# Aakash1312/Fluid-Simulation

Measured on AMD Instinct MI355X. Metric: simulated substeps/sec, higher is better.
Workload: dtype f64

## Files before the change

### fluid-simulation_amd/csrc/common.h

```cpp
#pragma once
#include <hip/hip_runtime.h>
#include <stdint.h>

namespace fl {

constexpr uint8_t F_SOLID = 1;
constexpr uint8_t F_FLUID = 2;
constexpr int F_CNT_SHIFT = 2;

struct Grid {
    int N;
    int lo;
    int hi;
    int nx, ny, nz;
    int ox, oy, oz;
    __host__ __device__ inline size_t idx(int ix, int iy, int iz) const
    {
        return ((size_t)ix * ny + (size_t)iy) * nz + (size_t)iz;
    }
    __host__ __device__ inline size_t cells() const { return (size_t)nx * ny * nz; }
    __host__ __device__ inline long sx() const { return (long)ny * nz; }
    __host__ __device__ inline int cx0() const { return lo + ox; }
    __host__ __device__ inline int cy0() const { return lo + oy; }
    __host__ __device__ inline int cz0() const { return lo + oz; }
// ... 167 lines not shown
    __host__ __device__ inline Particles shifted(long o) const
    {
        Particles q = *this;
        q.px += o; q.py += o; q.pz += o; q.vx += o; q.vy += o; q.vz += o; q.pid += o;
        return q;
    }
};
constexpr uint32_t PID_DEAD = 0xFFFFFFFFu;

void launch_bin_count(hipStream_t st, Grid g, long n, Particles p, int* key, int* slot, int* cell_count, int* part, StepState* ss);
void launch_bin_scatter(hipStream_t st, long n, const int* key, const int* slot, const int* cell_start, const uint32_t* pid, int* order,
                         uint32_t* spid);
void launch_bin_rank(hipStream_t st, long n_pos, long pos0, const int* key, const int* cell_start, const int* order, const uint32_t* spid,
                     int* order2);
void launch_reorder(hipStream_t st, long n, const int* order, Particles src, Particles dst, double* w = nullptr, long wstride = 0);
void launch_weights(hipStream_t st, long n, Particles p, double* w, long stride);
void launch_axpby_box(hipStream_t st, Grid g, Box box, double a, const double* x, double b, const double* y, double* out, const PcgState* gate = nullptr);
long p2g_max_items(Box box);
size_t p2g_part_doubles(Box box);
constexpr int P2G_PILED = 256;
void launch_p2g(hipStream_t st, Grid g, Box box, Particles p, const double* pw, long wstride, const int* cell_start, const uint8_t* flags,
                double* part, int* items, float* container, double* u, double* v, double* w, double* ub, double* vb, double* wb, int2* crowd_list = nullptr,
                Particles park = Particles{});
void launch_p2g_tiles(hipStream_t st, Grid g, Box box, Particles p, const double* pw, long wstride, const int* cell_start, const uint8_t* flags,
                      float* container, double* u, double* v, double* w, double* ub, double* vb, double* wb);
void launch_g2p_tiled(hipStream_t st, Grid g, Box pb, Particles p, const int* cell_start, const double* dcx, const double* dcy, const double* dcz,
                      const double* pcx, const double* pcy, const double* pcz, double blend, StepState* ss);
void launch_g2p(hipStream_t st, Grid g, long n, Particles p, const double* dcx, const double* dcy, const double* dcz, const double* pcx,
                const double* pcy, const double* pcz, double blend, StepState* ss);
void launch_advect(hipStream_t st, Grid g, long n, Particles p, const uint8_t* flags, double max_dt, double dx, StepState* ss);
void launch_advect_bin(hipStream_t st, Grid g, long n, Particles p, const uint8_t* flags, double max_dt, double dx, StepState* ss, int* key,
                       int* slot, int* cell_count, int* part);
void launch_pack_particles(hipStream_t st, long n, Particles p, double* pos_aos, double* vel_aos);
void launch_unpack_records(hipStream_t st, long n, const double* rec, Particles p, long off);
void launch_pack_records(hipStream_t st, long n, Particles p, long off, double* rec);
void launch_unpack_ids(hipStream_t st, long n, const double* pos, const double* vel, const uint32_t* ids, Particles p);
void launch_pack_ids(hipStream_t st, long n, Particles p, long off, double* pos, double* vel, uint32_t* ids);
void launch_unpack_particles(hipStream_t st, long n, const double* pos_aos, const double* vel_aos, Particles p);

void launch_out_mark(hipStream_t st, const float* f, int N, int off, int nl, int* flags);
void launch_out_pack(hipStream_t st, const float* f, int N, int lo, int off, int nl, const int* flags, const int* slot, float* values,
                     int* origin);
struct OutWin {
    int ny, nz;
    int ox, oy, oz;
    int olo[3], ohi[3];
    int lo, off;
    int l0[3], nl[3];
    __host__ __device__ inline long leaves() const { return (long)nl[0] * nl[1] * nl[2]; }
};
void launch_out_mark_win(hipStream_t st, const float* f, const OutWin& w, int* flags);
void launch_out_pack_win(hipStream_t st, const float* f, const OutWin& w, const int* flags, const int* slot, float* values, int* origin);
void launch_exclusive_scan(hipStream_t st, const int* in, int* out, long n, int* block_sums, int* total);
void launch_sort_tail(hipStream_t st, const int* cell_count, int* cell_start, long c1, long ncell);
void launch_index_scan(hipStream_t st, Grid g, const uint8_t* flags, int* indices, int* block_sums, int* total);
void launch_index_scan_flat(hipStream_t st, const uint8_t* flags, int* indices, long n, int* block_sums, int* total);
void launch_flags(hipStream_t st, Grid g, const uint8_t* solid, const float* container, uint8_t* flags, int x0, int x1);
void launch_index_scan_range(hipStream_t st, Grid g, const uint8_t* flags, int* indices, int* block_sums, int* total, int x0, int x1);
void launch_rhs_div(hipStream_t st, Grid g, Box box, const uint8_t* flags, const double* u, const double* v, const double* w,
                    float* rhs, float* diver, double dx, double gdt0, double gdt1, double gdt2, bool rows = false, const PcgState* gate = nullptr);
void launch_vel_update(hipStream_t st, Grid g, Box box, const uint8_t* flags, const double* p, double* u, double* v, double* w,
                       double k, double g0, double g1, double g2, bool rows = false, const PcgState* gate = nullptr);
void launch_flip_delta(hipStream_t st, Grid g, Box box, const double* u, const double* v, const double* w,
                       const double* ub, const double* vb, const double* wb, double* dcx, double* dcy, double* dcz, double* pcx, double* pcy, double* pcz);
void launch_err_norm(hipStream_t st, Grid g, Box box, const uint8_t* flags, const float* b, const float* b2, double* part, StepState* ss,
                     const PcgState* gate = nullptr);
void launch_zero_step_state(hipStream_t st, StepState* ss, int N);
struct ZeroList { float* f4[4]; double* f8[7]; };
void launch_zero_fields(hipStream_t st, const ZeroList& z, Grid g, Box box, bool rows = false);
// ... 128 lines not shown
```

### fluid-simulation_amd/csrc/fluid_api.hip

```cpp
#include "sim.h"
#include <algorithm>

using namespace fl;

static thread_local std::string g_err;
int fluid_fail(int code, const std::string& msg)
{
    g_err = msg;
    return code;
}
#define fail fluid_fail

Box fl::clip_dilate(const Box& b, int d, const Grid& g)
{
    Box r;
    r.x0 = b.x0 - d < 0 ? 0 : b.x0 - d;
    r.y0 = b.y0 - d < 0 ? 0 : b.y0 - d;
    r.z0 = b.z0 - d < 0 ? 0 : b.z0 - d;
    r.x1 = b.x1 + d > g.nx - 1 ? g.nx - 1 : b.x1 + d;
    r.y1 = b.y1 + d > g.ny - 1 ? g.ny - 1 : b.y1 + d;
    r.z1 = b.z1 + d > g.nz - 1 ? g.nz - 1 : b.z1 + d;
    return r;
}

// ... 189 lines not shown
    s->prm = *p;
    s->g = g;
    s->ncell = g.cells();
    s->dt = p->max_dt;
    s->mg_fp32 = p->mg_precision == FLUID_MG_FP32;
    s->warm = p->solve_start == FLUID_START_WARM;
    if (const char* e = getenv("FLUID_MG_CSWEEPS")) s->mg_csweeps = atoi(e);
    if (const char* e = getenv("FLUID_TILE_LISTS")) s->lists_force = atoi(e) != 0;
    if (const char* e = getenv("FLUID_P2G_FORM")) s->p2g_force = !strcmp(e, "rows") ? 1 : (!strcmp(e, "tiles") ? 2 : (!strcmp(e, "crowd") ? 3 : 0));
    if (const char* e = getenv("FLUID_MG_GALERKIN")) s->gal_mode = atoi(e);
    if (const char* e = getenv("FLUID_DROPLETS")) s->drops_on = atoi(e) != 0;
    if (const char* e = getenv("FLUID_ROW_SWEEPS")) s->row_sweeps = atoi(e) != 0;
    if (const char* e = getenv("FLUID_DROPLETS_MIN")) s->drop_min = atoi(e);
    if (const char* e = getenv("FLUID_ADVECT_BIN")) s->advect_bin = atoi(e) != 0;
    if (const char* e = getenv("FLUID_SOLVE_TAIL")) s->solve_tail = atoi(e) != 0;
    *out = nullptr;
    auto bail = [&](int rc) { fluid_destroy(s); return rc; };
#define A(expr) do { hipError_t e_ = (expr); if (e_ != hipSuccess) return bail(fail(FLUID_ERR_HIP, std::string(#expr) + ": " + hipGetErrorString(e_))); } while (0)
    A(hipStreamCreateWithFlags(&s->st, hipStreamNonBlocking));
    const size_t n = s->ncell;
    A(dalloc(&s->solid, n)); A(dalloc(&s->flags, n));
    A(dalloc(&s->container, n)); A(dalloc(&s->rhs, n)); A(dalloc(&s->diver, n)); A(dalloc(&s->diver2, n));
    A(dalloc(&s->u, n)); A(dalloc(&s->v, n)); A(dalloc(&s->w, n));
    A(dalloc(&s->ub, n)); A(dalloc(&s->vb, n)); A(dalloc(&s->wb, n));
    A(dalloc(&s->dcx, n)); A(dalloc(&s->dcy, n)); A(dalloc(&s->dcz, n));
    A(dalloc(&s->pressure, n));
    if (s->warm) {
        A(dalloc(&s->p_guess, n)); A(dalloc(&s->p_guess2, n));
        if (hipMemset(s->p_guess, 0, n * sizeof(double)) != hipSuccess || hipMemset(s->p_guess2, 0, n * sizeof(double)) != hipSuccess) return bail(FLUID_ERR_HIP);
        if (const char* e = getenv("FLUID_EXTRAPOLATE")) s->extrapolate = atoi(e) != 0;
        if (s->extrapolate) { A(dalloc(&s->p_q, n)); if (hipMemset(s->p_q, 0, n * sizeof(double)) != hipSuccess) return bail(FLUID_ERR_HIP); }
    }
    A(dalloc(&s->indices, n));
    A(dalloc(&s->scan_sums, (n + 2) / 2048 + 16));
// ... 155 lines not shown
    HIPCHK(hipMemcpyAsync(s->h_ss, s->ss, sizeof(StepState), hipMemcpyDeviceToHost, s->st));
    HIPCHK(hipStreamSynchronize(s->st));
    return FLUID_OK;
}

int fl::clear_dirty(fluid_sim* s)
{
    if (box_empty(s->dirty)) return FLUID_OK;
    const ZeroList z = {{s->container, s->rhs, s->diver, s->diver2}, {s->u, s->v, s->w, s->ub, s->vb, s->wb, s->pressure}};
    launch_zero_fields(s->st, z, s->g, s->dirty, !s->dist && s->row_sweeps);
    HIPCHK(hipGetLastError());
    s->dirty = Box{0, 0, 0, -1, -1, -1};
    return FLUID_OK;
}

int fl::sort_pass(fluid_sim* s, int ax0, int ax1, int* h_tail)
{
    const Grid g = s->g;
    const long ncell = (long)s->ncell, n2 = g.sx();
    const long c0 = (long)ax0 * n2, c1 = (long)(ax1 + 1) * n2;
    launch_zero_step_state(s->st, s->ss, g.N);
    HIPCHK(hipMemsetAsync(s->cell_count + c0, 0, (c1 - c0) * sizeof(int), s->st));
    HIPCHK(hipMemsetAsync(s->cell_count + ncell, 0, 4 * sizeof(int), s->st));
    launch_bin_count(s->st, g, s->np, s->pa.shifted(s->p_off), s->key, s->slot, s->cell_count, s->ipart, s->ss);
    launch_exclusive_scan(s->st, s->cell_count + c0, s->cell_start + c0, c1 - c0, s->scan_sums, s->cell_start + c1);
    launch_sort_tail(s->st, s->cell_count, s->cell_start, c1, ncell);
    launch_bin_scatter(s->st, s->np, s->key, s->slot, s->cell_start, s->pa.shifted(s->p_off).pid, s->order, s->spid);
    launch_bin_rank(s->st, s->np, 0, s->key, s->cell_start, s->order, s->spid, s->order2);
    HIPCHK(hipGetLastError());
    if (h_tail) HIPCHK(hipMemcpyAsync(h_tail, s->cell_start + ncell, 3 * sizeof(int), hipMemcpyDeviceToHost, s->st));
    return read_ss(s);
}

static int sort_binned(fluid_sim* s)
{
    const Grid g = s->g;
    const long ncell = (long)s->ncell, n2 = g.sx();
    const long c0 = (long)s->bin_x0 * n2, c1 = (long)(s->bin_x1 + 1) * n2;
    launch_zero_step_state(s->st, s->ss, g.N);
    launch_exclusive_scan(s->st, s->cell_count + c0, s->cell_start + c0, c1 - c0, s->scan_sums, s->cell_start + c1);
    launch_sort_tail(s->st, s->cell_count, s->cell_start, c1, ncell);
    launch_bin_scatter(s->st, s->np, s->key, s->slot, s->cell_start, s->pa.shifted(s->p_off).pid, s->order, s->spid);
    launch_bin_rank(s->st, s->np, 0, s->key, s->cell_start, s->order, s->spid, s->order2);
    HIPCHK(hipGetLastError());
    StepState& h = *s->h_ss;
    for (int a = 0; a < 3; ++a) h.bbox_min[a] = s->bin_min[a], h.bbox_max[a] = s->bin_max[a];
    h.n_out = s->bin_n_out;
    h.max_cell = s->bin_max_cell;
    return FLUID_OK;
}

static int phase_sort(fluid_sim* s)
{
    const Grid g = s->g;
    int tok = prof_begin(s, FLUID_PROF_SORT, (double)s->np);
    int ax0 = 0, ax1 = g.nx - 1;
    const bool guess = s->sort_hint && !box_empty(s->Pb);
    if (guess) {
// ... 18 lines not shown
    s->sort_hint = true;
    s->n_out = s->h_ss->n_out;
    s->max_cell = s->h_ss->max_cell;
    const StepState& h = *s->h_ss;
    if (h.bbox_max[0] < 0) {
        s->Pb = Box{0, 0, 0, -1, -1, -1};
    } else {
        s->Pb = Box{h.bbox_min[0], h.bbox_min[1], h.bbox_min[2], h.bbox_max[0], h.bbox_max[1], h.bbox_max[2]};
    }
    if (!box_empty(s->Pb)) {
        s->Rb = clip_dilate(s->Pb, 1, g);
        s->Sb = clip_dilate(s->Pb, 2, g);
    } else {
        s->Rb = s->Sb = s->Pb;
    }
    launch_reorder(s->st, s->np, s->order2, s->pa.shifted(s->p_off), s->pb, s->pw, s->cap);
    HIPCHK(hipGetLastError());
    std::swap(s->pa, s->pb);
    s->p_off = 0;
    prof_end(s, FLUID_PROF_SORT, tok);
    s->sorted = true;
    return FLUID_OK;
}

int fl::run_p2g(fluid_sim* s, const Box& box)
{
    const long ref_cells = s->p2g_ref_cells > 0 ? s->p2g_ref_cells : s->Rb.cells();
    const bool airy = s->last_num_active > 0 && (double)s->last_num_active < 0.3 * (double)ref_cells;
    const bool huge = (size_t)12 * sizeof(double) * (size_t)box.cells() > ((size_t)16 << 30);
    const bool piled = s->max_cell > P2G_PILED || airy;
    if (s->p2g_force ? s->p2g_force == 2 : huge) {
// ... 642 lines not shown
        HIPCHK(hipMalloc((void**)q, s->ncell * sizeof(double)));
        HIPCHK(hipMemsetAsync(*q, 0, s->ncell * sizeof(double), s->st));
    }
    return FLUID_OK;
}

static int phase_flip_advect(fluid_sim* s)
{
    if (!s->have_p2g) return fail(FLUID_ERR_STATE, "flip_advect before p2g");
    HIPCHK(hipSetDevice(s->prm.device));
    int rcp = pic_fields(s);
    if (rcp) return rcp;
    if (!box_empty(s->Rb)) launch_flip_delta(s->st, s->g, s->Rb, s->u, s->v, s->w, s->ub, s->vb, s->wb, s->dcx, s->dcy, s->dcz, s->pcx, s->pcy, s->pcz);
    int tok = prof_begin(s, FLUID_PROF_G2P, (double)s->np);
    if (s->sorted && s->p_off == 0 && (double)s->np >= 4.0 * (double)s->Pb.cells()) {
        launch_g2p_tiled(s->st, s->g, s->Pb, s->pa, s->cell_start, s->dcx, s->dcy, s->dcz, s->pcx, s->pcy, s->pcz, s->prm.flip_blend, s->ss);
        if (!box_empty(s->Pb)) s->stats.paths |= FLUID_PATH_G2P_TILES;
        if (s->n_out > 0)
            launch_g2p(s->st, s->g, s->n_out, s->pa.shifted(s->np - s->n_out), s->dcx, s->dcy, s->dcz, s->pcx, s->pcy, s->pcz, s->prm.flip_blend, s->ss);
    } else {
        launch_g2p(s->st, s->g, s->np, s->pa.shifted(s->p_off), s->dcx, s->dcy, s->dcz, s->pcx, s->pcy, s->pcz, s->prm.flip_blend, s->ss);
    }
    prof_end(s, FLUID_PROF_G2P, tok);
    const bool bin = s->advect_bin && !s->dist && s->np > 0 && s->sorted && s->sort_hint && !box_empty(s->Pb);
    s->binned = false;
    if (bin) {
        const Grid g = s->g;
        s->bin_x0 = std::max(0, s->Pb.x0 - 3);
        s->bin_x1 = std::min(g.nx - 1, s->Pb.x1 + 3);
        const long n2 = g.sx(), c0 = (long)s->bin_x0 * n2, c1 = (long)(s->bin_x1 + 1) * n2;
        HIPCHK(hipMemsetAsync(s->cell_count + c0, 0, (c1 - c0) * sizeof(int), s->st));
        HIPCHK(hipMemsetAsync(s->cell_count + s->ncell, 0, 4 * sizeof(int), s->st));
        launch_advect_bin(s->st, g, s->np, s->pa.shifted(s->p_off), s->flags, s->prm.max_dt, s->prm.dx, s->ss, s->key, s->slot, s->cell_count, s->ipart);
    } else {
        launch_advect(s->st, s->g, s->np, s->pa.shifted(s->p_off), s->flags, s->prm.max_dt, s->prm.dx, s->ss);
    }
    HIPCHK(hipGetLastError());
    int rc = read_ss(s);
    if (rc) return rc;
    if (bin) {
        const StepState& h = *s->h_ss;
        for (int a = 0; a < 3; ++a) s->bin_min[a] = h.bbox_min[a], s->bin_max[a] = h.bbox_max[a];
        s->bin_n_out = h.n_out;
        s->bin_max_cell = h.max_cell;
        s->binned = true;
    }
    s->dt = s->h_ss->dt;
// ... 373 lines not shown
```

### fluid-simulation_amd/csrc/fluid_dist.hip

```cpp
#include "sim.h"
#include "dist_kernels.h"

using namespace fl;
#define fail fluid_fail
int cuts_from_hist(int n, const int64_t* hist, int P, int32_t* cuts);

#define COMMCHK(expr)                                                                              \
    do {                                                                                           \
        if ((expr) != 0) return fail(FLUID_ERR_HIP, std::string("comm callback failed: ") + #expr); \
    } while (0)

namespace {

constexpr int HALO_W = 4;

struct IBox {
    int lo[3], hi[3];
};
inline bool ib_empty(const IBox& b) { return b.hi[0] <= b.lo[0] || b.hi[1] <= b.lo[1] || b.hi[2] <= b.lo[2]; }
inline IBox ib_isect(const IBox& a, const IBox& b)
{
    IBox r;
    for (int k = 0; k < 3; ++k) { r.lo[k] = std::max(a.lo[k], b.lo[k]); r.hi[k] = std::min(a.hi[k], b.hi[k]); }
    if (ib_empty(r)) for (int k = 0; k < 3; ++k) { r.lo[k] = a.lo[k]; r.hi[k] = a.lo[k]; }
// ... 398 lines not shown
        s->stats.box_hi[a] = d->Rg.hi[a] - 1;
    }
}

int dist_g2p_advect(fluid_sim* s, fluid_step_stats_t* stats)
{
    DistState* d = s->ds;
    const Grid g = s->g;
    int rc;
    launch_kill_ghosts(s->st, g, d->ob, s->np, s->pa.shifted(s->p_off));
    int tok = prof_begin(s, FLUID_PROF_G2P, (double)s->np);
    const IBox ownb{{d->ob.lo[0], d->ob.lo[1], d->ob.lo[2]}, {d->ob.hi[0], d->ob.hi[1], d->ob.hi[2]}};
    const int org[3] = {g.ox, g.oy, g.oz};
    const Box ownPb = to_box(ib_isect(d->Pg, ownb), org);
    if (s->p_off == 0 && !box_empty(ownPb) && (double)s->np >= 4.0 * (double)ownPb.cells()) {
        launch_g2p_tiled(s->st, g, ownPb, s->pa, s->cell_start, s->dcx, s->dcy, s->dcz, s->pcx, s->pcy, s->pcz, s->prm.flip_blend, s->ss);
        if (s->n_out > 0)
            launch_g2p(s->st, g, s->n_out, s->pa.shifted(s->np - s->n_out), s->dcx, s->dcy, s->dcz, s->pcx, s->pcy, s->pcz, s->prm.flip_blend, s->ss);
    } else {
        launch_g2p(s->st, g, s->np, s->pa.shifted(s->p_off), s->dcx, s->dcy, s->dcz, s->pcx, s->pcy, s->pcz, s->prm.flip_blend, s->ss);
    }
    prof_end(s, FLUID_PROF_G2P, tok);
    HIPCHK(hipGetLastError());
    if ((rc = comm_allreduce(s, &s->ss->max_speed_bits, 1, FLUID_DT_I64, FLUID_OP_MAX))) return rc;
    launch_advect(s->st, g, s->np, s->pa.shifted(s->p_off), s->flags, s->prm.max_dt, s->prm.dx, s->ss);
    HIPCHK(hipGetLastError());
    if ((rc = read_ss(s))) return rc;
    s->dt = s->h_ss->dt;
    double ms;
    memcpy(&ms, &s->h_ss->max_speed_bits, sizeof(double));
    s->stats.max_speed = ms;
// ... 1561 lines not shown
```

### fluid-simulation_amd/csrc/kernels_grid.hip

```cpp
#include "common.h"

namespace fl {

constexpr int SCAN_T = 256;
constexpr int SCAN_E = 8;
constexpr int SCAN_CHUNK = SCAN_T * SCAN_E;

template <int MODE>
__device__ __forceinline__ int scan_load(const void* in, long i)
{
    if (MODE == 0) return ((const int*)in)[i];
    return (((const uint8_t*)in)[i] & F_FLUID) ? 1 : 0;
}

template <int MODE, bool VEC>
__device__ __forceinline__ void scan_load8(const void* in, long base, long n, int v[SCAN_E])
{
    if (VEC && base >= 0 && base + SCAN_E <= n) {
        if (MODE == 0) {
            const int4 a = *(const int4*)((const int*)in + base), b = *(const int4*)((const int*)in + base + 4);
            v[0] = a.x; v[1] = a.y; v[2] = a.z; v[3] = a.w;
            v[4] = b.x; v[5] = b.y; v[6] = b.z; v[7] = b.w;
        } else {
            const uint2 w = *(const uint2*)((const uint8_t*)in + base);
// ... 492 lines not shown
{
    ss->bbox_min[0] = ss->bbox_min[1] = ss->bbox_min[2] = N;
    ss->bbox_max[0] = ss->bbox_max[1] = ss->bbox_max[2] = -1;
    ss->num_active = 0;
    ss->n_out = 0;
    ss->n_drop_fail = 0;
    ss->max_speed_bits = 0ull;
    ss->err_num = 0;
    ss->err_den = 0;
}
void launch_zero_step_state(hipStream_t st, StepState* ss, int N)
{
    hipLaunchKernelGGL(k_zero_step_state, dim3(1), dim3(1), 0, st, ss, N);
}

__global__ void k_sort_tail(const int* __restrict__ cell_count, int* __restrict__ cell_start, long c1, long ncell)
{
    const int t = cell_start[c1];
    cell_start[ncell] = t;
    cell_start[ncell + 1] = t + cell_count[ncell];
    cell_start[ncell + 2] = t + cell_count[ncell] + cell_count[ncell + 1];
}
void launch_sort_tail(hipStream_t st, const int* cell_count, int* cell_start, long c1, long ncell)
{
    hipLaunchKernelGGL(k_sort_tail, dim3(1), dim3(1), 0, st, cell_count, cell_start, c1, ncell);
}

__global__ __launch_bounds__(256) void k_zero_fields(ZeroList z, Grid g, Box box)
{
    const int a = blockIdx.y;
    float* pf = z.f4[0];
#pragma unroll
    for (int q = 1; q < 4; ++q) pf = (a == q) ? z.f4[q] : pf;
    double* pd = z.f8[0];
#pragma unroll
    for (int q = 1; q < 7; ++q) pd = (a - 4 == q) ? z.f8[q] : pd;
    CellIt it = box_cell(g, box);
    if (!it.ok) return;
// ... 170 lines not shown
```

### fluid-simulation_amd/csrc/kernels_particles.hip

```cpp
#include "common.h"

namespace fl {

struct BinAcc {
    int mn[3] = {0x7fffffff, 0x7fffffff, 0x7fffffff}, mx[3] = {-1, -1, -1};
    int nout = 0, cmax = 0;
};
__device__ __forceinline__ void bin_one(const Grid& g, long ncell, long i, double px, double py, double pz, bool dead, int* __restrict__ key,
                                        int* __restrict__ slot, int* __restrict__ cell_count, BinAcc& acc)
{
    int bx = (int)round(px) - g.cx0(), by = (int)round(py) - g.cy0(), bz = (int)round(pz) - g.cz0();
    bool in = bx >= 0 && bx < g.nx && by >= 0 && by < g.ny && bz >= 0 && bz < g.nz;
    int k = in ? (int)g.idx(bx, by, bz) : (int)ncell;
    if (dead) { k = (int)ncell + 1; in = false; }
    key[i] = k;
    {
        const int lane = threadIdx.x & 63;
        const int kp = __shfl_up(k, 1, 64);
        const bool head = lane == 0 || kp != k;
        const unsigned long long hm = __ballot(head);
        const unsigned long long below = hm & ((2ull << lane) - 1ull);
        const int start = 63 - __clzll((long long)below);
        const unsigned long long above = (lane == 63) ? 0ull : (hm >> (lane + 1)) << (lane + 1);
        const unsigned long long act = __ballot(true);
// ... 161 lines not shown
        for (int d = 0; d < 3; ++d) w[(a * 3 + d) * stride + j] = spline_at(q[a], b - 1 + d, d);
    }
}

__global__ __launch_bounds__(256) void k_reorder(long n, const int* __restrict__ order, Particles s, Particles d, double* __restrict__ w,
                                                 long wstride)
{
    long j = (long)blockIdx.x * 256 + threadIdx.x;
    if (j >= n) return;
    int i = order[j];
    const double px = s.px[i], py = s.py[i], pz = s.pz[i];
    d.px[j] = px; d.py[j] = py; d.pz[j] = pz;
    d.vx[j] = s.vx[i]; d.vy[j] = s.vy[i]; d.vz[j] = s.vz[i];
    d.pid[j] = s.pid[i];
    if (w) axis_weights(px, py, pz, w, wstride, j);
}

__global__ __launch_bounds__(256) void k_weights(long n, Particles p, double* __restrict__ w, long stride)
{
    long j = (long)blockIdx.x * 256 + threadIdx.x;
    if (j >= n) return;
    axis_weights(p.px[j], p.py[j], p.pz[j], w, stride, j);
}

constexpr int P2G_SLOTS = 256 * 4;
constexpr int P2G_THREADS = 192;
constexpr int P2G_CH = 384;
constexpr int P2G_SEG = P2G_CH / 8 + 1;
__device__ __forceinline__ int p2g_slot(int k) { return (k & 7) * P2G_SEG + (k >> 3); }
constexpr int P2G_LDS = 8 * P2G_SEG;
// ... 541 lines not shown
            p.vx[i] = vx; p.vy[i] = vy; p.vz[i] = vz;
        }
        len = sqrt(vx * vx + vy * vy + vz * vz);
        if (!(len == len)) len = 0;
    }
    len = wave_max(len);
    if ((threadIdx.x & 63) == 0) sm[threadIdx.x >> 6] = len;
    __syncthreads();
    if (threadIdx.x == 0) {
        double m = sm[0];
        for (int k = 1; k < 4; ++k) m = sm[k] > m ? sm[k] : m;
        if (m > 0) atomicMax(&ss->max_speed_bits, (unsigned long long)__double_as_longlong(m));
    }
}

constexpr int G2P_TX = 4, G2P_TY = 4, G2P_TZ = 30;
template <bool PIC>
__global__ __launch_bounds__(256) void k_g2p_tiled(Grid g, Box pb, Particles p, const int* __restrict__ cell_start,
                                                   const double* __restrict__ dcx, const double* __restrict__ dcy,
                                                   const double* __restrict__ dcz, const double* __restrict__ pcx,
                                                   const double* __restrict__ pcy, const double* __restrict__ pcz, double blend, StepState* ss)
{
    constexpr int LX = G2P_TX + 2, LY = G2P_TY + 2, LZ = G2P_TZ + 2, LN = LX * LY * LZ, NROW = G2P_TX * G2P_TY;
    __shared__ double sf[PIC ? 6 : 3][LN];
    __shared__ int srow[NROW][2];
    __shared__ double sm[4];
    const int tid = threadIdx.x;
    const int nty = (pb.ny() + G2P_TY - 1) / G2P_TY, ntz = (pb.nz() + G2P_TZ - 1) / G2P_TZ;
    const int tile = blockIdx.x;
    const int tz = tile % ntz, ty = (tile / ntz) % nty, tx = tile / (ntz * nty);
    const int x0 = pb.x0 + tx * G2P_TX, y0 = pb.y0 + ty * G2P_TY, z0 = pb.z0 + tz * G2P_TZ;
    const int z1 = z0 + G2P_TZ - 1 < pb.z1 ? z0 + G2P_TZ - 1 : pb.z1;
    if (tid < NROW) {
        const int cx = x0 + tid / G2P_TY, cy = y0 + tid % G2P_TY;
        int a = 0, b = 0;
        if (cx <= pb.x1 && cy <= pb.y1) {
            a = cell_start[g.idx(cx, cy, z0)];
            b = cell_start[g.idx(cx, cy, z1) + 1];
        }
        srow[tid][0] = a;
        srow[tid][1] = b;
    }
    for (int t = tid; t < LN; t += 256) {
        const int lx = t / (LY * LZ), r = t - lx * (LY * LZ), ly = r / LZ, lz = r - ly * LZ;
        const int gx = x0 - 1 + lx, gy = y0 - 1 + ly, gz = z0 - 1 + lz;
        const bool in = gx >= 0 && gx < g.nx && gy >= 0 && gy < g.ny && gz >= 0 && gz < g.nz;
        const size_t c = in ? g.idx(gx, gy, gz) : 0;
        sf[0][t] = in ? dcx[c] : 0.0;
        sf[1][t] = in ? dcy[c] : 0.0;
        sf[2][t] = in ? dcz[c] : 0.0;
        if (PIC) {
            sf[PIC ? 3 : 0][t] = in ? pcx[c] : 0.0;
            sf[PIC ? 4 : 0][t] = in ? pcy[c] : 0.0;
            sf[PIC ? 5 : 0][t] = in ? pcz[c] : 0.0;
        }
    }
    __syncthreads();
    const int wlo = g.lo + 2, whi = g.hi - 2;
    double len = 0;
    for (int row = 0; row < NROW; ++row) {
        const int a = srow[row][0], b = srow[row][1];
        for (int i = a + tid; i < b; i += 256) {
            const double cx = p.px[i], cy = p.py[i], cz = p.pz[i];
            const int fcx = (int)round(cx), fcy = (int)round(cy), fcz = (int)round(cz);
            double wx[3], wy[3], wz[3];
#pragma unroll
            for (int d = 0; d < 3; ++d) {
                const int ax = fcx - 1 + d, ay = fcy - 1 + d, az = fcz - 1 + d;
                wx[d] = (ax >= wlo && ax <= whi) ? spline_at(cx, ax, d) : 0.0;
                wy[d] = (ay >= wlo && ay <= whi) ? spline_at(cy, ay, d) : 0.0;
                wz[d] = (az >= wlo && az <= whi) ? spline_at(cz, az, d) : 0.0;
            }
            const int lb = ((fcx - g.cx0() - x0) * LY + (fcy - g.cy0() - y0)) * LZ + (fcz - g.cz0() - z0);
            double weight = 0, d0 = 0, d1 = 0, d2 = 0, q0 = 0, q1 = 0, q2 = 0;
#pragma unroll
            for (int xi = 0; xi < 3; ++xi)
#pragma unroll
// ... 175 lines not shown
}
void launch_bin_scatter(hipStream_t st, long n, const int* key, const int* slot, const int* cell_start, const uint32_t* pid, int* order,
                         uint32_t* spid)
{
    if (n > 0) hipLaunchKernelGGL(k_bin_scatter, dim3(nblk(n)), dim3(256), 0, st, n, key, slot, cell_start, pid, order, spid);
}
void launch_bin_rank(hipStream_t st, long n_pos, long pos0, const int* key, const int* cell_start, const int* order, const uint32_t* spid,
                     int* order2)
{
    if (n_pos > 0) hipLaunchKernelGGL(k_bin_rank, dim3(nblk(n_pos)), dim3(256), 0, st, n_pos, pos0, key, cell_start, order, spid, order2);
}
void launch_reorder(hipStream_t st, long n, const int* order, Particles src, Particles dst, double* w, long wstride)
{
    if (n > 0) hipLaunchKernelGGL(k_reorder, dim3(nblk(n)), dim3(256), 0, st, n, order, src, dst, w, wstride);
}
void launch_weights(hipStream_t st, long n, Particles p, double* w, long stride)
{
    if (n > 0) hipLaunchKernelGGL(k_weights, dim3(nblk(n)), dim3(256), 0, st, n, p, w, stride);
}
static void p2g_cut(const Box& box, int& ntz, int& zt, int& nseg)
{
    ntz = (box.nz() + P2G_ZT - 1) / P2G_ZT;
    zt = (box.nz() + ntz - 1) / ntz;
    nseg = 1;
    long best = -1;
    const long per = (long)(box.nx() + 2) * ntz;
    for (int k = 1; k <= box.ny(); ++k) {
        const long ys = (box.ny() + k - 1) / k, rounds = (per * k + P2G_SLOTS - 1) / P2G_SLOTS, cost = rounds * (ys + 2);
        if (best < 0 || cost < best) { best = cost; nseg = k; }
    }
// ... 29 lines not shown
        hipLaunchKernelGGL(k_p2g_crowd_list, dim3(nblk((long)sb.nx() * sb.ny() * ((sb.nz() + 3) / 4))), dim3(256), 0, st, g, sb, cell_start, crowd_list, items + 1);
        hipLaunchKernelGGL(k_p2g_crowd_sum, dim3(2048), dim3(64 * PC_WAVES), 0, st, p, pw, wstride, crowd_list, items + 1, park);
        if (vec) hipLaunchKernelGGL((k_p2g_rows<true, true>), dim3(nt), dim3(P2G_THREADS), 0, st, g, box, p, pw, wstride, cell_start, part, cells, zt, items, park, colflag, ntz);
        else hipLaunchKernelGGL((k_p2g_rows<false, true>), dim3(nt), dim3(P2G_THREADS), 0, st, g, box, p, pw, wstride, cell_start, part, cells, zt, items, park, colflag, ntz);
    } else if (vec) hipLaunchKernelGGL((k_p2g_rows<true, false>), dim3(nt), dim3(P2G_THREADS), 0, st, g, box, p, pw, wstride, cell_start, part, cells, zt, items, park, colflag, ntz);
    else hipLaunchKernelGGL((k_p2g_rows<false, false>), dim3(nt), dim3(P2G_THREADS), 0, st, g, box, p, pw, wstride, cell_start, part, cells, zt, items, park, colflag, ntz);
    hipLaunchKernelGGL(k_p2g_combine, dim3(nblk(cells)), dim3(256), 0, st, g, box, part, cells, flags, container, u, v, w, ub, vb, wb, items, colflag, zt, ntz);
}
void launch_p2g_tiles(hipStream_t st, Grid g, Box box, Particles p, const double* pw, long wstride, const int* cell_start, const uint8_t* flags,
                      float* container, double* u, double* v, double* w, double* ub, double* vb, double* wb)
{
    const int ntz = (box.nz() + P2G_ZT - 1) / P2G_ZT, zt = (box.nz() + ntz - 1) / ntz;
    const unsigned nt = (unsigned)(((box.nx() + P2GT_T - 1) / P2GT_T) * ((box.ny() + P2GT_T - 1) / P2GT_T) * ntz);
    hipLaunchKernelGGL(k_p2g_tiles, dim3(nt), dim3(P2GT_THREADS), 0, st, g, box, p, pw, wstride, cell_start, flags, container, u, v, w, ub, vb, wb, zt);
}
void launch_g2p_tiled(hipStream_t st, Grid g, Box pb, Particles p, const int* cell_start, const double* dcx, const double* dcy, const double* dcz,
                      const double* pcx, const double* pcy, const double* pcz, double blend, StepState* ss)
{
    if (pb.cells() <= 0) return;
    const unsigned nt = (unsigned)(((pb.nx() + G2P_TX - 1) / G2P_TX) * ((pb.ny() + G2P_TY - 1) / G2P_TY) * ((pb.nz() + G2P_TZ - 1) / G2P_TZ));
    if (pcx) hipLaunchKernelGGL(k_g2p_tiled<true>, dim3(nt), dim3(256), 0, st, g, pb, p, cell_start, dcx, dcy, dcz, pcx, pcy, pcz, blend, ss);
    else hipLaunchKernelGGL(k_g2p_tiled<false>, dim3(nt), dim3(256), 0, st, g, pb, p, cell_start, dcx, dcy, dcz, pcx, pcy, pcz, blend, ss);
}
void launch_g2p(hipStream_t st, Grid g, long n, Particles p, const double* dcx, const double* dcy, const double* dcz, const double* pcx,
                const double* pcy, const double* pcz, double blend, StepState* ss)
{
    if (n > 0) hipLaunchKernelGGL(k_g2p, dim3(nblk(n)), dim3(256), 0, st, g, n, p, dcx, dcy, dcz, pcx, pcy, pcz, blend, ss);
}
void launch_advect(hipStream_t st, Grid g, long n, Particles p, const uint8_t* flags, double max_dt, double dx, StepState* ss)
{
    if (n > 0) hipLaunchKernelGGL(k_advect, dim3(nblk(n)), dim3(256), 0, st, g, n, p, flags, max_dt, dx, ss);
    hipLaunchKernelGGL(k_publish_dt, dim3(1), dim3(1), 0, st, max_dt, dx, ss, (const int*)nullptr, 0);
}
void launch_advect_bin(hipStream_t st, Grid g, long n, Particles p, const uint8_t* flags, double max_dt, double dx, StepState* ss, int* key,
                       int* slot, int* cell_count, int* part)
{
    unsigned nb = nblk(n);
// ... 31 lines not shown
```

### fluid-simulation_amd/csrc/sim.h

```cpp
#pragma once
#include "common.h"
#include "../../include/fluid_hip.h"

#include <cmath>
#include <cstdio>
#include <cstdlib>
#include <cstring>
#include <string>
#include <utility>
#include <vector>

int fluid_fail(int code, const std::string& msg);
#define HIPCHK(expr)                                                                                              \
    do {                                                                                                          \
        hipError_t e_ = (expr);                                                                                   \
        if (e_ != hipSuccess)                                                                                     \
            return fluid_fail(FLUID_ERR_HIP, std::string(#expr) + ": " + hipGetErrorString(e_) + " @" + std::to_string(__LINE__)); \
    } while (0)

using namespace fl;

struct ProfClass {
    long launches = 0, sampled = 0;
    double ms = 0, cells = 0;
// ... 85 lines not shown
    long p2g_ref_cells = 0;
    long last_num_active = 0;
    StepState* ss = nullptr;
    StepState* h_ss = nullptr;
    Box Pb{0, 0, 0, -1, -1, -1}, Rb{0, 0, 0, -1, -1, -1}, Sb{0, 0, 0, -1, -1, -1};
    Box dirty{0, 0, 0, -1, -1, -1};
    int flag_x0 = 0, flag_x1 = -1;
    bool flags_valid = false;
    bool sorted = false, have_p2g = false, have_flags = false;
    long n_out = 0;
    bool sort_hint = false;
    bool advect_bin = true;
    bool binned = false;
    int bin_x0 = 0, bin_x1 = -1;
    int bin_min[3] = {0, 0, 0}, bin_max[3] = {-1, -1, -1}, bin_n_out = 0, bin_max_cell = 0;
    bool solve_tail = true;
    bool tail_ran = false;
    double dt = 0.1;
    fluid_step_stats_t stats{};
    static constexpr int MG_MAXL = 8;
    int mg_nl = 0, mg_tail = 0;
    long mg_last_iters_k[3] = {0, 0, 0};
    int pass_class() const { return stats.outer_passes < 2 ? stats.outer_passes : 2; }
    int mg_csweeps = 3;
    MLevel mgl[MG_MAXL];
    uint8_t *mg_typ[MG_MAXL] = {}, *mg_cnt[MG_MAXL] = {};
    int gal_mode = 1;
    int gal_it[2] = {-1, -1};
    int gal_since_probe = 0;
    bool gal_eligible = false;
// ... 84 lines not shown
```

Before: 155.0.

## Fuse bin rank into reorder, add occupancy-driven G2P tile depth, flatten G2P row loop

```diff
diff --git a/fluid-simulation_amd/csrc/common.h b/fluid-simulation_amd/csrc/common.h
--- a/fluid-simulation_amd/csrc/common.h
+++ b/fluid-simulation_amd/csrc/common.h
@@ -205,6 +205,8 @@
 void launch_bin_rank(hipStream_t st, long n_pos, long pos0, const int* key, const int* cell_start, const int* order, const uint32_t* spid,
                      int* order2);
 void launch_reorder(hipStream_t st, long n, const int* order, Particles src, Particles dst, double* w = nullptr, long wstride = 0);
+void launch_rank_reorder(hipStream_t st, long n, const int* key, const int* cell_start, const int* order, const uint32_t* spid, Particles src,
+                         Particles dst, double* w, long wstride);
 void launch_weights(hipStream_t st, long n, Particles p, double* w, long stride);
 void launch_axpby_box(hipStream_t st, Grid g, Box box, double a, const double* x, double b, const double* y, double* out, const PcgState* gate = nullptr);
 long p2g_max_items(Box box);
@@ -215,8 +217,16 @@
                 Particles park = Particles{});
 void launch_p2g_tiles(hipStream_t st, Grid g, Box box, Particles p, const double* pw, long wstride, const int* cell_start, const uint8_t* flags,
                       float* container, double* u, double* v, double* w, double* ub, double* vb, double* wb);
-void launch_g2p_tiled(hipStream_t st, Grid g, Box pb, Particles p, const int* cell_start, const double* dcx, const double* dcy, const double* dcz,
-                      const double* pcx, const double* pcy, const double* pcz, double blend, StepState* ss);
+constexpr int G2P_NDEPTH = 4;
+constexpr int G2P_DEPTHS[G2P_NDEPTH] = {10, 13, 18, 30};
+struct G2pPlan {
+    int slots[2][G2P_NDEPTH] = {};
+    int force = 0;
+};
+int g2p_plan_init(G2pPlan* pl, int device);
+int g2p_depth(const G2pPlan& pl, Box pb, long np, bool pic);
+void launch_g2p_tiled(hipStream_t st, Grid g, Box pb, long np, const G2pPlan& plan, Particles p, const int* cell_start, const double* dcx,
+                      const double* dcy, const double* dcz, const double* pcx, const double* pcy, const double* pcz, double blend, StepState* ss);
 void launch_g2p(hipStream_t st, Grid g, long n, Particles p, const double* dcx, const double* dcy, const double* dcz, const double* pcx,
                 const double* pcy, const double* pcz, double blend, StepState* ss);
 void launch_advect(hipStream_t st, Grid g, long n, Particles p, const uint8_t* flags, double max_dt, double dx, StepState* ss);
@@ -243,7 +253,7 @@
 void launch_out_mark_win(hipStream_t st, const float* f, const OutWin& w, int* flags);
 void launch_out_pack_win(hipStream_t st, const float* f, const OutWin& w, const int* flags, const int* slot, float* values, int* origin);
 void launch_exclusive_scan(hipStream_t st, const int* in, int* out, long n, int* block_sums, int* total);
-void launch_sort_tail(hipStream_t st, const int* cell_count, int* cell_start, long c1, long ncell);
+void launch_sort_tail(hipStream_t st, int* cell_count, int* cell_start, long c1, long ncell);
 void launch_index_scan(hipStream_t st, Grid g, const uint8_t* flags, int* indices, int* block_sums, int* total);
 void launch_index_scan_flat(hipStream_t st, const uint8_t* flags, int* indices, long n, int* block_sums, int* total);
 void launch_flags(hipStream_t st, Grid g, const uint8_t* solid, const float* container, uint8_t* flags, int x0, int x1);
diff --git a/fluid-simulation_amd/csrc/fluid_api.hip b/fluid-simulation_amd/csrc/fluid_api.hip
--- a/fluid-simulation_amd/csrc/fluid_api.hip
+++ b/fluid-simulation_amd/csrc/fluid_api.hip
@@ -227,10 +227,17 @@
     if (const char* e = getenv("FLUID_DROPLETS_MIN")) s->drop_min = atoi(e);
     if (const char* e = getenv("FLUID_ADVECT_BIN")) s->advect_bin = atoi(e) != 0;
     if (const char* e = getenv("FLUID_SOLVE_TAIL")) s->solve_tail = atoi(e) != 0;
+    if (const char* e = getenv("FLUID_RANK_REORDER")) s->rank_reorder = atoi(e) != 0;
+    if (const char* e = getenv("FLUID_G2P_TZ")) s->g2p_plan.force = atoi(e);
     *out = nullptr;
     auto bail = [&](int rc) { fluid_destroy(s); return rc; };
 #define A(expr) do { hipError_t e_ = (expr); if (e_ != hipSuccess) return bail(fail(FLUID_ERR_HIP, std::string(#expr) + ": " + hipGetErrorString(e_))); } while (0)
     A(hipStreamCreateWithFlags(&s->st, hipStreamNonBlocking));
+    if (g2p_plan_init(&s->g2p_plan, p->device)) return bail(fail(FLUID_ERR_HIP, "no occupancy figure for k_g2p_tiled"));
+    if (getenv("FLUID_G2P_PRINT")) {
+        for (int k = 0; k < G2P_NDEPTH; ++k)
+            fprintf(stderr, "k_g2p_tiled depth %d: %d resident blocks (FLIP), %d (PIC)\n", G2P_DEPTHS[k], s->g2p_plan.slots[0][k], s->g2p_plan.slots[1][k]);
+    }
     const size_t n = s->ncell;
     A(dalloc(&s->solid, n)); A(dalloc(&s->flags, n));
     A(dalloc(&s->container, n)); A(dalloc(&s->rhs, n)); A(dalloc(&s->diver, n)); A(dalloc(&s->diver2, n));
@@ -416,6 +423,8 @@
     return FLUID_OK;
 }
 
+static inline bool fused_rank(const fluid_sim* s) { return s->rank_reorder && !s->dist; }
+
 int fl::sort_pass(fluid_sim* s, int ax0, int ax1, int* h_tail)
 {
     const Grid g = s->g;
@@ -428,7 +437,7 @@
     launch_exclusive_scan(s->st, s->cell_count + c0, s->cell_start + c0, c1 - c0, s->scan_sums, s->cell_start + c1);
     launch_sort_tail(s->st, s->cell_count, s->cell_start, c1, ncell);
     launch_bin_scatter(s->st, s->np, s->key, s->slot, s->cell_start, s->pa.shifted(s->p_off).pid, s->order, s->spid);
-    launch_bin_rank(s->st, s->np, 0, s->key, s->cell_start, s->order, s->spid, s->order2);
+    if (!fused_rank(s)) launch_bin_rank(s->st, s->np, 0, s->key, s->cell_start, s->order, s->spid, s->order2);
     HIPCHK(hipGetLastError());
     if (h_tail) HIPCHK(hipMemcpyAsync(h_tail, s->cell_start + ncell, 3 * sizeof(int), hipMemcpyDeviceToHost, s->st));
     return read_ss(s);
@@ -443,7 +452,7 @@
     launch_exclusive_scan(s->st, s->cell_count + c0, s->cell_start + c0, c1 - c0, s->scan_sums, s->cell_start + c1);
     launch_sort_tail(s->st, s->cell_count, s->cell_start, c1, ncell);
     launch_bin_scatter(s->st, s->np, s->key, s->slot, s->cell_start, s->pa.shifted(s->p_off).pid, s->order, s->spid);
-    launch_bin_rank(s->st, s->np, 0, s->key, s->cell_start, s->order, s->spid, s->order2);
+    if (!fused_rank(s)) launch_bin_rank(s->st, s->np, 0, s->key, s->cell_start, s->order, s->spid, s->order2);
     HIPCHK(hipGetLastError());
     StepState& h = *s->h_ss;
     for (int a = 0; a < 3; ++a) h.bbox_min[a] = s->bin_min[a], h.bbox_max[a] = s->bin_max[a];
@@ -492,7 +501,8 @@
     } else {
         s->Rb = s->Sb = s->Pb;
     }
-    launch_reorder(s->st, s->np, s->order2, s->pa.shifted(s->p_off), s->pb, s->pw, s->cap);
+    if (fused_rank(s)) launch_rank_reorder(s->st, s->np, s->key, s->cell_start, s->order, s->spid, s->pa.shifted(s->p_off), s->pb, s->pw, s->cap);
+    else launch_reorder(s->st, s->np, s->order2, s->pa.shifted(s->p_off), s->pb, s->pw, s->cap);
     HIPCHK(hipGetLastError());
     std::swap(s->pa, s->pb);
     s->p_off = 0;
@@ -1165,7 +1175,7 @@
     if (!box_empty(s->Rb)) launch_flip_delta(s->st, s->g, s->Rb, s->u, s->v, s->w, s->ub, s->vb, s->wb, s->dcx, s->dcy, s->dcz, s->pcx, s->pcy, s->pcz);
     int tok = prof_begin(s, FLUID_PROF_G2P, (double)s->np);
     if (s->sorted && s->p_off == 0 && (double)s->np >= 4.0 * (double)s->Pb.cells()) {
-        launch_g2p_tiled(s->st, s->g, s->Pb, s->pa, s->cell_start, s->dcx, s->dcy, s->dcz, s->pcx, s->pcy, s->pcz, s->prm.flip_blend, s->ss);
+        launch_g2p_tiled(s->st, s->g, s->Pb, s->np, s->g2p_plan, s->pa, s->cell_start, s->dcx, s->dcy, s->dcz, s->pcx, s->pcy, s->pcz, s->prm.flip_blend, s->ss);
         if (!box_empty(s->Pb)) s->stats.paths |= FLUID_PATH_G2P_TILES;
         if (s->n_out > 0)
             launch_g2p(s->st, s->g, s->n_out, s->pa.shifted(s->np - s->n_out), s->dcx, s->dcy, s->dcz, s->pcx, s->pcy, s->pcz, s->prm.flip_blend, s->ss);
@@ -1181,7 +1191,6 @@
         s->bin_x1 = std::min(g.nx - 1, s->Pb.x1 + 3);
         const long n2 = g.sx(), c0 = (long)s->bin_x0 * n2, c1 = (long)(s->bin_x1 + 1) * n2;
         HIPCHK(hipMemsetAsync(s->cell_count + c0, 0, (c1 - c0) * sizeof(int), s->st));
-        HIPCHK(hipMemsetAsync(s->cell_count + s->ncell, 0, 4 * sizeof(int), s->st));
         launch_advect_bin(s->st, g, s->np, s->pa.shifted(s->p_off), s->flags, s->prm.max_dt, s->prm.dx, s->ss, s->key, s->slot, s->cell_count, s->ipart);
     } else {
         launch_advect(s->st, s->g, s->np, s->pa.shifted(s->p_off), s->flags, s->prm.max_dt, s->prm.dx, s->ss);
diff --git a/fluid-simulation_amd/csrc/fluid_dist.hip b/fluid-simulation_amd/csrc/fluid_dist.hip
--- a/fluid-simulation_amd/csrc/fluid_dist.hip
+++ b/fluid-simulation_amd/csrc/fluid_dist.hip
@@ -436,7 +436,7 @@
     const int org[3] = {g.ox, g.oy, g.oz};
     const Box ownPb = to_box(ib_isect(d->Pg, ownb), org);
     if (s->p_off == 0 && !box_empty(ownPb) && (double)s->np >= 4.0 * (double)ownPb.cells()) {
-        launch_g2p_tiled(s->st, g, ownPb, s->pa, s->cell_start, s->dcx, s->dcy, s->dcz, s->pcx, s->pcy, s->pcz, s->prm.flip_blend, s->ss);
+        launch_g2p_tiled(s->st, g, ownPb, s->np, s->g2p_plan, s->pa, s->cell_start, s->dcx, s->dcy, s->dcz, s->pcx, s->pcy, s->pcz, s->prm.flip_blend, s->ss);
         if (s->n_out > 0)
             launch_g2p(s->st, g, s->n_out, s->pa.shifted(s->np - s->n_out), s->dcx, s->dcy, s->dcz, s->pcx, s->pcy, s->pcz, s->prm.flip_blend, s->ss);
     } else {
diff --git a/fluid-simulation_amd/csrc/kernels_grid.hip b/fluid-simulation_amd/csrc/kernels_grid.hip
--- a/fluid-simulation_amd/csrc/kernels_grid.hip
+++ b/fluid-simulation_amd/csrc/kernels_grid.hip
@@ -530,14 +530,16 @@
     hipLaunchKernelGGL(k_zero_step_state, dim3(1), dim3(1), 0, st, ss, N);
 }
 
-__global__ void k_sort_tail(const int* __restrict__ cell_count, int* __restrict__ cell_start, long c1, long ncell)
+__global__ void k_sort_tail(int* __restrict__ cell_count, int* __restrict__ cell_start, long c1, long ncell)
 {
     const int t = cell_start[c1];
+    const int n0 = cell_count[ncell], n1 = cell_count[ncell + 1];
     cell_start[ncell] = t;
-    cell_start[ncell + 1] = t + cell_count[ncell];
-    cell_start[ncell + 2] = t + cell_count[ncell] + cell_count[ncell + 1];
-}
-void launch_sort_tail(hipStream_t st, const int* cell_count, int* cell_start, long c1, long ncell)
+    cell_start[ncell + 1] = t + n0;
+    cell_start[ncell + 2] = t + n0 + n1;
+    cell_count[ncell] = cell_count[ncell + 1] = cell_count[ncell + 2] = cell_count[ncell + 3] = 0;
+}
+void launch_sort_tail(hipStream_t st, int* cell_count, int* cell_start, long c1, long ncell)
 {
     hipLaunchKernelGGL(k_sort_tail, dim3(1), dim3(1), 0, st, cell_count, cell_start, c1, ncell);
 }
diff --git a/fluid-simulation_amd/csrc/kernels_particles.hip b/fluid-simulation_amd/csrc/kernels_particles.hip
--- a/fluid-simulation_amd/csrc/kernels_particles.hip
+++ b/fluid-simulation_amd/csrc/kernels_particles.hip
@@ -199,6 +199,47 @@
     d.vx[j] = s.vx[i]; d.vy[j] = s.vy[i]; d.vz[j] = s.vz[i];
     d.pid[j] = s.pid[i];
     if (w) axis_weights(px, py, pz, w, wstride, j);
+}
+
+__global__ __launch_bounds__(256) void k_rank_reorder(long n, const int* __restrict__ key, const int* __restrict__ cell_start,
+                                                      const int* __restrict__ order, const uint32_t* __restrict__ spid, Particles s, Particles d,
+                                                      double* __restrict__ w, long wstride)
+{
+    __shared__ uint32_t sid[RANK_CH];
+    __shared__ int sAB[2];
+    const long j = (long)blockIdx.x * 256 + threadIdx.x;
+    const bool act = j < n;
+    int a = 0, b = 0;
+    uint32_t mine = 0;
+    double px = 0, py = 0, pz = 0, vx = 0, vy = 0, vz = 0;
+    if (act) {
+        const int src = order[j];
+        const int k = key[src];
+        px = s.px[src]; py = s.py[src]; pz = s.pz[src];
+        vx = s.vx[src]; vy = s.vy[src]; vz = s.vz[src];
+        a = cell_start[k];
+        b = cell_start[k + 1];
+        mine = spid[j];
+    }
+    if (threadIdx.x == 0) sAB[0] = a;
+    if (act && (j + 1 == n || threadIdx.x == 255)) sAB[1] = b;
+    __syncthreads();
+    const int A = sAB[0], B = sAB[1];
+    int rank = 0;
+    for (int c0 = A; c0 < B; c0 += RANK_CH) {
+        const int c1 = c0 + RANK_CH < B ? c0 + RANK_CH : B;
+        if (c0 != A) __syncthreads();
+        for (int t = c0 + threadIdx.x; t < c1; t += 256) sid[t - c0] = spid[t];
+        __syncthreads();
+        const int lo = a > c0 ? a : c0, hi = b < c1 ? b : c1;
+        for (int t = lo; t < hi; ++t) rank += sid[t - c0] < mine;
+    }
+    if (!act) return;
+    const long dst = (long)a + rank;
+    d.px[dst] = px; d.py[dst] = py; d.pz[dst] = pz;
+    d.vx[dst] = vx; d.vy[dst] = vy; d.vz[dst] = vz;
+    d.pid[dst] = mine;
+    if (w) axis_weights(px, py, pz, w, wstride, dst);
 }
 
 __global__ __launch_bounds__(256) void k_weights(long n, Particles p, double* __restrict__ w, long stride)
@@ -770,16 +811,18 @@
     }
 }
 
-constexpr int G2P_TX = 4, G2P_TY = 4, G2P_TZ = 30;
-template <bool PIC>
+constexpr int G2P_TX = 4, G2P_TY = 4;
+template <bool PIC, int G2P_TZ>
 __global__ __launch_bounds__(256) void k_g2p_tiled(Grid g, Box pb, Particles p, const int* __restrict__ cell_start,
                                                    const double* __restrict__ dcx, const double* __restrict__ dcy,
                                                    const double* __restrict__ dcz, const double* __restrict__ pcx,
                                                    const double* __restrict__ pcy, const double* __restrict__ pcz, double blend, StepState* ss)
 {
     constexpr int LX = G2P_TX + 2, LY = G2P_TY + 2, LZ = G2P_TZ + 2, LN = LX * LY * LZ, NROW = G2P_TX * G2P_TY;
+    static_assert(NROW == 16, "the row search below takes 4 halving steps");
     __shared__ double sf[PIC ? 6 : 3][LN];
-    __shared__ int srow[NROW][2];
+    __shared__ int srow[NROW];
+    __shared__ int spre[NROW + 1];
     __shared__ double sm[4];
     const int tid = threadIdx.x;
     const int nty = (pb.ny() + G2P_TY - 1) / G2P_TY, ntz = (pb.nz() + G2P_TZ - 1) / G2P_TZ;
@@ -787,15 +830,24 @@
     const int tz = tile % ntz, ty = (tile / ntz) % nty, tx = tile / (ntz * nty);
     const int x0 = pb.x0 + tx * G2P_TX, y0 = pb.y0 + ty * G2P_TY, z0 = pb.z0 + tz * G2P_TZ;
     const int z1 = z0 + G2P_TZ - 1 < pb.z1 ? z0 + G2P_TZ - 1 : pb.z1;
-    if (tid < NROW) {
+    if (tid < 64) {
         const int cx = x0 + tid / G2P_TY, cy = y0 + tid % G2P_TY;
         int a = 0, b = 0;
-        if (cx <= pb.x1 && cy <= pb.y1) {
+        if (tid < NROW && cx <= pb.x1 && cy <= pb.y1) {
             a = cell_start[g.idx(cx, cy, z0)];
             b = cell_start[g.idx(cx, cy, z1) + 1];
         }
-        srow[tid][0] = a;
-        srow[tid][1] = b;
+        int incl = b - a;
+#pragma unroll
+        for (int o = 1; o < NROW; o <<= 1) {
+            const int t = __shfl_up(incl, o, 64);
+            if (tid >= o) incl += t;
+        }
+        if (tid < NROW) {
+            srow[tid] = a;
+            spre[tid] = incl - (b - a);
+            if (tid == NROW - 1) spre[NROW] = incl;
+        }
     }
     for (int t = tid; t < LN; t += 256) {
         const int lx = t / (LY * LZ), r = t - lx * (LY * LZ), ly = r / LZ, lz = r - ly * LZ;
@@ -814,9 +866,14 @@
     __syncthreads();
     const int wlo = g.lo + 2, whi = g.hi - 2;
     double len = 0;
-    for (int row = 0; row < NROW; ++row) {
-        const int a = srow[row][0], b = srow[row][1];
-        for (int i = a + tid; i < b; i += 256) {
+    const int ntile = spre[NROW];
+    {
+        for (int f = tid; f < ntile; f += 256) {
+            int row = spre[8] <= f ? 8 : 0;
+            row += spre[row + 4] <= f ? 4 : 0;
+            row += spre[row + 2] <= f ? 2 : 0;
+            row += spre[row + 1] <= f ? 1 : 0;
+            const int i = srow[row] + (f - spre[row]);
             const double cx = p.px[i], cy = p.py[i], cz = p.pz[i];
             const int fcx = (int)round(cx), fcy = (int)round(cy), fcz = (int)round(cz);
             double wx[3], wy[3], wz[3];
@@ -1022,6 +1079,11 @@
 {
     if (n > 0) hipLaunchKernelGGL(k_reorder, dim3(nblk(n)), dim3(256), 0, st, n, order, src, dst, w, wstride);
 }
+void launch_rank_reorder(hipStream_t st, long n, const int* key, const int* cell_start, const int* order, const uint32_t* spid, Particles src,
+                         Particles dst, double* w, long wstride)
+{
+    if (n > 0) hipLaunchKernelGGL(k_rank_reorder, dim3(nblk(n)), dim3(256), 0, st, n, key, cell_start, order, spid, src, dst, w, wstride);
+}
 void launch_weights(hipStream_t st, long n, Particles p, double* w, long stride)
 {
     if (n > 0) hipLaunchKernelGGL(k_weights, dim3(nblk(n)), dim3(256), 0, st, n, p, w, stride);
@@ -1081,13 +1143,73 @@
     const unsigned nt = (unsigned)(((box.nx() + P2GT_T - 1) / P2GT_T) * ((box.ny() + P2GT_T - 1) / P2GT_T) * ntz);
     hipLaunchKernelGGL(k_p2g_tiles, dim3(nt), dim3(P2GT_THREADS), 0, st, g, box, p, pw, wstride, cell_start, flags, container, u, v, w, ub, vb, wb, zt);
 }
-void launch_g2p_tiled(hipStream_t st, Grid g, Box pb, Particles p, const int* cell_start, const double* dcx, const double* dcy, const double* dcz,
-                      const double* pcx, const double* pcy, const double* pcz, double blend, StepState* ss)
+template <bool PIC, int TZ>
+static int g2p_slots_of(int cus, int* out)
+{
+    int nb = 0;
+    if (hipOccupancyMaxActiveBlocksPerMultiprocessor(&nb, k_g2p_tiled<PIC, TZ>, 256, 0) != hipSuccess || nb <= 0) return -1;
+    *out = nb * cus;
+    return 0;
+}
+template <int K>
+static int g2p_slots_all(int cus, G2pPlan* pl)
+{
+    if constexpr (K < G2P_NDEPTH)
+        return g2p_slots_of<false, G2P_DEPTHS[K]>(cus, &pl->slots[0][K]) | g2p_slots_of<true, G2P_DEPTHS[K]>(cus, &pl->slots[1][K]) |
+               g2p_slots_all<K + 1>(cus, pl);
+    else
+        return 0;
+}
+int g2p_plan_init(G2pPlan* pl, int device)
+{
+    int cus = 0;
+    if (hipDeviceGetAttribute(&cus, hipDeviceAttributeMultiprocessorCount, device) != hipSuccess || cus <= 0) return -1;
+    return g2p_slots_all<0>(cus, pl);
+}
+constexpr int G2P_PCOST = 8;
+int g2p_depth(const G2pPlan& pl, Box pb, long np, bool pic)
+{
+    if (pl.force > 0)
+        for (int k = 0; k < G2P_NDEPTH; ++k)
+            if (G2P_DEPTHS[k] == pl.force) return k;
+    const long cells = pb.cells() > 0 ? pb.cells() : 1;
+    const long ncol = (long)((pb.nx() + G2P_TX - 1) / G2P_TX) * ((pb.ny() + G2P_TY - 1) / G2P_TY);
+    int best = G2P_NDEPTH - 1;
+    double best_cost = -1;
+    for (int k = G2P_NDEPTH - 1; k >= 0; --k) {
+        const int d = G2P_DEPTHS[k], slots = pl.slots[pic ? 1 : 0][k];
+        if (slots <= 0) continue;
+        const long nt = ncol * ((pb.nz() + d - 1) / d);
+        const double rounds = nt <= slots ? 1.0 : (double)nt / slots + 0.5;
+        const int deep = d < pb.nz() ? d : pb.nz();
+        const double tile = (double)G2P_PCOST * G2P_TX * G2P_TY * deep * ((double)np / (double)cells) + (double)(G2P_TX + 2) * (G2P_TY + 2) * (d + 2);
+        const double cost = rounds * tile;
+        if (best_cost < 0 || cost < best_cost) { best_cost = cost; best = k; }
+    }
+    return best;
+}
+template <int TZ>
+static void g2p_tiled_go(hipStream_t st, Grid g, Box pb, Particles p, const int* cell_start, const double* dcx, const double* dcy, const double* dcz,
+                         const double* pcx, const double* pcy, const double* pcz, double blend, StepState* ss)
+{
+    const unsigned nt = (unsigned)(((pb.nx() + G2P_TX - 1) / G2P_TX) * ((pb.ny() + G2P_TY - 1) / G2P_TY) * ((pb.nz() + TZ - 1) / TZ));
+    if (pcx) hipLaunchKernelGGL((k_g2p_tiled<true, TZ>), dim3(nt), dim3(256), 0, st, g, pb, p, cell_start, dcx, dcy, dcz, pcx, pcy, pcz, blend, ss);
+    else hipLaunchKernelGGL((k_g2p_tiled<false, TZ>), dim3(nt), dim3(256), 0, st, g, pb, p, cell_start, dcx, dcy, dcz, pcx, pcy, pcz, blend, ss);
+}
+template <int K>
+static void g2p_tiled_pick(int k, hipStream_t st, Grid g, Box pb, Particles p, const int* cell_start, const double* dcx, const double* dcy,
+                           const double* dcz, const double* pcx, const double* pcy, const double* pcz, double blend, StepState* ss)
+{
+    if constexpr (K < G2P_NDEPTH) {
+        if (k == K) g2p_tiled_go<G2P_DEPTHS[K]>(st, g, pb, p, cell_start, dcx, dcy, dcz, pcx, pcy, pcz, blend, ss);
+        else g2p_tiled_pick<K + 1>(k, st, g, pb, p, cell_start, dcx, dcy, dcz, pcx, pcy, pcz, blend, ss);
+    }
+}
+void launch_g2p_tiled(hipStream_t st, Grid g, Box pb, long np, const G2pPlan& plan, Particles p, const int* cell_start, const double* dcx,
+                      const double* dcy, const double* dcz, const double* pcx, const double* pcy, const double* pcz, double blend, StepState* ss)
 {
     if (pb.cells() <= 0) return;
-    const unsigned nt = (unsigned)(((pb.nx() + G2P_TX - 1) / G2P_TX) * ((pb.ny() + G2P_TY - 1) / G2P_TY) * ((pb.nz() + G2P_TZ - 1) / G2P_TZ));
-    if (pcx) hipLaunchKernelGGL(k_g2p_tiled<true>, dim3(nt), dim3(256), 0, st, g, pb, p, cell_start, dcx, dcy, dcz, pcx, pcy, pcz, blend, ss);
-    else hipLaunchKernelGGL(k_g2p_tiled<false>, dim3(nt), dim3(256), 0, st, g, pb, p, cell_start, dcx, dcy, dcz, pcx, pcy, pcz, blend, ss);
+    g2p_tiled_pick<0>(g2p_depth(plan, pb, np, pcx != nullptr), st, g, pb, p, cell_start, dcx, dcy, dcz, pcx, pcy, pcz, blend, ss);
 }
 void launch_g2p(hipStream_t st, Grid g, long n, Particles p, const double* dcx, const double* dcy, const double* dcz, const double* pcx,
                 const double* pcy, const double* pcz, double blend, StepState* ss)
diff --git a/fluid-simulation_amd/csrc/sim.h b/fluid-simulation_amd/csrc/sim.h
--- a/fluid-simulation_amd/csrc/sim.h
+++ b/fluid-simulation_amd/csrc/sim.h
@@ -123,6 +123,8 @@
     bool binned = false;
     int bin_x0 = 0, bin_x1 = -1;
     int bin_min[3] = {0, 0, 0}, bin_max[3] = {-1, -1, -1}, bin_n_out = 0, bin_max_cell = 0;
+    bool rank_reorder = true;
+    G2pPlan g2p_plan;
     bool solve_tail = true;
     bool tail_ran = false;
     double dt = 0.1;
```

After: 155.2, median of 6. No clear change (+0.2%).
